# craftsangjae/instance-segmentation-road-project

Measured on AMD Instinct MI355X. Metric: images/sec at 1024x1024 (MaskLab inference hot path, full forward), higher is better.
Workload: dtype f32

## Files before the change

### include/masklab_hip.h

```cpp
#ifndef MASKLAB_HIP_H
#define MASKLAB_HIP_H

#include <stdint.h>

#ifdef __cplusplus
extern "C" {
#endif

#define ML_OK 0
#define ML_E_BADARG (-1)
#define ML_E_LAUNCH (-2)
#define ML_E_NOGPU  (-3)

enum { ML_ACT_NONE = 0, ML_ACT_RELU = 1, ML_ACT_RELU6 = 2, ML_ACT_SIGMOID = 3 };
enum { ML_MATH_F32 = 0, ML_MATH_F16 = 1, ML_MATH_F16S = 2, ML_MATH_F32X3 = 3 };

#define ML_ABI_VERSION 7
int ml_version(void);
const char *ml_last_error(void);
int ml_device_check(void);

typedef struct ml_conv2d_desc {
    const float *in;
    const float *wgt;
    const float *bias;
    const float *residual;
    float *out;
    int32_t B, H, W;
    int32_t in_cstride, in_coff;
    int32_t span;
    int32_t span_pad;
    int32_t cpp_shift;
    int32_t Ho, Wo;
    int32_t KH, KW, stride, dil, pad_t, pad_l;
    int32_t cout;
    int32_t n_pad;
    int32_t out_cstride, out_coff;
    int32_t res_cstride, res_coff;
    int32_t act;
    int32_t group_cin_step;
    int32_t shuffle2x2;
    int32_t tile;
    int32_t math;
    int32_t out_f16;
    int64_t out_bstride;
    const int32_t *live;
    int32_t live_period;
    int32_t reserved1;
    double *gn_partials;
} ml_conv2d_desc;

int ml_conv2d_f32(const ml_conv2d_desc *d, void *stream);

#define ML_CONV_MAX_PROBLEMS 12
int64_t ml_conv2d_workspace_bytes(void);
int ml_conv2d_multi_f32(const ml_conv2d_desc *descs, int32_t n, void *workspace, int64_t workspace_bytes,
                        void *stream);
int ml_conv2d_ntile(int32_t cout, int32_t tile);
int ml_conv2d_launch_ntile(const ml_conv2d_desc *descs, int32_t n, int32_t has_workspace);
int ml_conv2d_launch_mtile(const ml_conv2d_desc *descs, int32_t n, int32_t has_workspace);
int ml_conv2d_uses_pipe(const ml_conv2d_desc *d);
int ml_conv2d_launch_splits(const ml_conv2d_desc *descs, int32_t n, int64_t workspace_bytes, int32_t *splits);
int ml_conv2d_wino_eligible(const ml_conv2d_desc *d);
int ml_conv2d_wino_narrow(const ml_conv2d_desc *d);
int64_t ml_conv2d_gn_min_launch_tiles(void);

#define ML_CONV_WGRAD_MAX_PROBLEMS 8
typedef struct ml_conv2d_wgrad_desc {
    ml_conv2d_desc conv;
    float *dkernel;
    float *dbias;
    const float *add_kernel;
    const float *add_bias;
} ml_conv2d_wgrad_desc;
int ml_conv2d_wgrad_multi_f32(const ml_conv2d_wgrad_desc *descs, int32_t n, void *workspace, int64_t workspace_bytes,
                              void *stream);
int ml_conv2d_wgrad_plan(const ml_conv2d_wgrad_desc *desc, int32_t *slices, int32_t *slice_pixels, int64_t *workspace_bytes);
int ml_conv2d_grad_gather_dy_f32(const float *dy, float *out, int32_t B, int32_t HW, int32_t cout, int32_t dy_cstride,
                                 int64_t dy_bstride, void *stream);

int ml_gconv3x3_f32(const float *in, const float *wgt, const float *bias, float *out,
                    int32_t B, int32_t H, int32_t W, int32_t C, int32_t c, int32_t Ho, int32_t Wo,
                    int32_t stride, int32_t pad_t, int32_t pad_l, int32_t act, void *stream);

int ml_gconv3x3_f16(const void *in, const float *wgt, const float *bias, void *out,
                    int32_t B, int32_t H, int32_t W, int32_t C, int32_t c, int32_t Ho, int32_t Wo,
                    int32_t stride, int32_t pad_t, int32_t pad_l, int32_t act, void *stream);

int ml_gconv3x3_launch_plan(int32_t B, int32_t H, int32_t W, int32_t C, int32_t c, int32_t stride, int32_t Ho, int32_t Wo,
                            int32_t is_half, int32_t plan[6]);

int ml_maxpool3x3s2_f16(const void *in, void *out, int32_t B, int32_t H, int32_t W, int32_t C,
                        int32_t Ho, int32_t Wo, int32_t pad_t, int32_t pad_l, void *stream);
int ml_subsample2_f16(const void *in, void *out, int32_t B, int32_t H, int32_t W, int32_t C, void *stream);
int ml_cast_f16_to_f32(const void *in, float *out, int64_t n, void *stream);
int ml_cast_f32_to_f16(const float *in, void *out, int64_t n, void *stream);
int ml_resize_bilinear_ac_f16(const void *in, const void *add, void *out,
                              int32_t B, int32_t H, int32_t W, int32_t C, int32_t in_cstride, int32_t in_coff,
                              int32_t Ho, int32_t Wo, int32_t add_cstride, int32_t add_coff,
                              int32_t out_cstride, int32_t out_coff, void *stream);
int ml_dwconv3x3_f16(const void *in, const float *wgt, const float *bias, void *out,
                     int32_t B, int32_t H, int32_t W, int32_t C, int32_t in_cstride, int32_t in_coff,
                     int32_t out_cstride, int32_t out_coff, int32_t Ho, int32_t Wo,
                     int32_t stride, int32_t dil, int32_t pad_t, int32_t pad_l, int32_t act, void *stream);
int ml_global_mean_f16(const void *in, void *out, int32_t B, int32_t HW, int32_t C, void *stream);

int ml_stem7x7s2_pool_f16(const float *image, const void *wgt_h, const float *bias, void *out, int32_t B, int32_t H,
                          int32_t W, int32_t Hp, int32_t Wp, void *stream);
int ml_stem7x7s2_pool_f32(const float *image, const float *wgt, const float *bias, float *out, int32_t B, int32_t H,
                          int32_t W, int32_t Hp, int32_t Wp, void *stream);
int ml_stem7x7s2_pool_x3(const float *image, const void *wgt_x3, const float *bias, float *out, int32_t B, int32_t H,
                         int32_t W, int32_t Hp, int32_t Wp, void *stream);

typedef struct ml_deconv_out_problem {
    const float *x, *wd, *bd, *wo_table, *bo;
    float *out;
    int64_t M;
// ... 373 lines not shown
```

### instance-segmentation-road-project_amd/csrc/conv_wino.hip

```cpp
#include "gfx_mem.h"

namespace {

constexpr int WMAXP = ML_CONV_MAX_PROBLEMS;
constexpr int WT = 64;
constexpr int WN = 64;
constexpr int WK = 8;
constexpr int WCHUNK = WK * 32 * 16;
constexpr int WSTEP = 4 * 32 * 16;
constexpr int NSLOT_P = 3;
constexpr int SLOT_P = WT * 16 * 8;
constexpr int NSLOT_W = 4;
constexpr int SLOT_W = 2 * WSTEP;
constexpr int RING_W = NSLOT_P * SLOT_P;
constexpr int LDS_BYTES = (RING_W + NSLOT_W * SLOT_W) * 4;
static_assert(LDS_BYTES == 160 * 1024, "the two rings fill the CU's LDS");
#ifndef WINO_EXP
#define WINO_EXP 0
#endif
constexpr unsigned OOB = 0x80000000u;
constexpr long long SPAN_MAX = 0x7fffff00ll;

struct WProblem {
    ml_conv2d_desc d;
    int TH, TW, T;
    int MB, NB, nchunks;
};

struct WArgs {
    int n;
    int start[WMAXP + 1];
    WProblem p[WMAXP];
};

typedef f32x4 f32x4d __attribute__((aligned(4)));

__device__ __forceinline__ void out_store(float *base, float *ptr, float val) {
#if (WINO_EXP & 8) && defined(__HIP_DEVICE_COMPILE__)
    const __amdgpu_buffer_rsrc_t none = rsrc_bytes(base, 0);
    __builtin_amdgcn_raw_buffer_store_b32(__builtin_bit_cast(unsigned, val), none, (int)((ptr - base) * 4), 0, 0);
#else
    *ptr = val;
#endif
}
__device__ __forceinline__ void out_store(float *base, float *ptr, f32x4 val) {
#if (WINO_EXP & 8) && defined(__HIP_DEVICE_COMPILE__)
    const __amdgpu_buffer_rsrc_t none = rsrc_bytes(base, 0);
    __builtin_amdgcn_raw_buffer_store_b128(__builtin_bit_cast(u32x4, val), none, (int)((ptr - base) * 4), 0, 0);
#else
    *reinterpret_cast<f32x4d *>(ptr) = val;
#endif
}

__device__ __forceinline__ void bt_d_b_op(int k, const float d[16], float t[16], float v[16]) {
    if (k < 16) {
        const int j = k >> 2;
        switch (k & 3) {
            case 0: t[0 * 4 + j] = d[0 * 4 + j] - d[2 * 4 + j]; break;
            case 1: t[1 * 4 + j] = d[1 * 4 + j] + d[2 * 4 + j]; break;
            case 2: t[2 * 4 + j] = d[2 * 4 + j] - d[1 * 4 + j]; break;
            default: t[3 * 4 + j] = d[1 * 4 + j] - d[3 * 4 + j]; break;
        }
    } else {
        const int i = (k - 16) >> 2;
        switch (k & 3) {
            case 0: v[i * 4 + 0] = t[i * 4 + 0] - t[i * 4 + 2]; break;
            case 1: v[i * 4 + 1] = t[i * 4 + 1] + t[i * 4 + 2]; break;
            case 2: v[i * 4 + 2] = t[i * 4 + 2] - t[i * 4 + 1]; break;
            default: v[i * 4 + 3] = t[i * 4 + 1] - t[i * 4 + 3]; break;
        }
    }
}

__global__ void __launch_bounds__(512, 1) conv_wino_kernel(const WArgs args) {
    extern __shared__ __align__(16) float lds[];

    int pi = 0;
    while (pi + 1 < args.n && (int)blockIdx.x >= args.start[pi + 1]) ++pi;
    const WProblem &P = args.p[pi];
    const ml_conv2d_desc &p = P.d;
    const int b = (int)blockIdx.x - args.start[pi];
    const int g = b / (8 * P.NB), rr = b - g * 8 * P.NB;
    const int nt2 = rr >> 3;
    const int mt = g * 8 + (rr & 7);
    if (mt >= P.MB) return;
    if (p.live) {
        const int lv = max(1, *p.live), tpi0 = P.TH * P.TW;
        const int b0 = mt * WT / tpi0, b1 = min(mt * WT + WT, P.T) - 1;
        bool any = false;
        for (int bi = b0; bi <= b1 / tpi0 && !any; ++bi) any = bi % p.live_period < lv;
        if (!any) return;
    }

    const int tid = threadIdx.x, lane = tid & 63;
    const int wave = __builtin_amdgcn_readfirstlane(tid >> 6);
    const int tg = wave & 3, h = wave >> 2;
    const int r = lane & 15, kq = lane >> 4;
    const int tpi = P.TH * P.TW;

    const int gt0 = mt * WT;
    long long base_pix;
    {
        const int bi = gt0 / tpi, rem = gt0 - bi * tpi, ty = rem / P.TW;
        base_pix = ((long long)bi * p.H + max(2 * ty - 1, 0)) * p.W;
    }
    const size_t cstride = (size_t)p.in_cstride;
    const float *pin = p.in + p.in_coff + (size_t)base_pix * cstride;
    int voff_p[4];
    {
        const int rt = (lane >> 1) & 15;
        const int quad = (lane & 1) ^ ((rt >> 2) & 1);
        const int gt = gt0 + (wave >> 1) * 16 + rt;
        int bi = 0, ty = 0, tx = 0;
        if (gt < P.T) {
            bi = gt / tpi;
            const int rem = gt - bi * tpi;
            ty = rem / P.TW;
            tx = rem - ty * P.TW;
        }
#pragma unroll
        for (int i = 0; i < 4; ++i) {
            const int px = 8 * (wave & 1) + 2 * i + (lane >> 5);
            const int y = 2 * ty - 1 + (px >> 2), x = 2 * tx - 1 + (px & 3);
            voff_p[i] = (int)OOB;
            if (gt < P.T && y >= 0 && y < p.H && x >= 0 && x < p.W)
                voff_p[i] = (int)((((long long)bi * p.H + y) * p.W + x - base_pix) * (long long)cstride * 4) + quad * 16;
        }
    }
    const int voff_w = ((wave & 3) * 512 + r * 16 + kq * 4) * 4;
    const float *wsrc = p.wgt + (size_t)(2 * nt2 + (wave >> 2)) * P.nchunks * WCHUNK;
    float *dst_p = lds + (wave >> 1) * 2048 + (wave & 1) * 1024;
    float *dst_w = lds + RING_W + (wave >> 2) * WSTEP + (wave & 3) * 512;
    const int nch = P.nchunks, nsteps = 2 * P.nchunks;
    const bool dead = (2 * nt2 + h) * 32 >= p.cout;

    auto rsrc_p = [&](int j) __attribute__((always_inline)) {
        const bool real = j < nch && !(WINO_EXP & 1);
        return rsrc_bytes(pin + j * 8, real ? (int)OOB : 0);
    };
    auto rsrc_w = [&](int s) __attribute__((always_inline)) {
        const bool real = s < nsteps && !dead && !(WINO_EXP & 2);
        return rsrc_bytes(wsrc + (size_t)s * WSTEP, real ? WSTEP * 4 : 0);
    };

    f32x4 acc[2][16];
#pragma unroll
    for (int t = 0; t < 2; ++t)
#pragma unroll
        for (int q = 0; q < 16; ++q) acc[t][q] = f32x4{0.f, 0.f, 0.f, 0.f};

    const float *pa_lane0 = lds + tg * 2048 + r * 8 + 4 * ((r >> 2) & 1) + kq;
    const float *pa_lane1 = lds + tg * 2048 + r * 8 + 4 * (((r >> 2) & 1) ^ 1) + kq;
    const float *pb_lane = lds + RING_W + h * WSTEP + kq * 512 + r * 4;
    struct Ops {
        float d[16], t[16], v[16];
        f32x4 b[2][4];
    };
    auto read_ops = [&](const float *pa, const float *pb, Ops &o) __attribute__((always_inline)) {
#pragma unroll
        for (int t = 0; t < 2; ++t)
#pragma unroll
            for (int pq = 0; pq < 4; ++pq) o.b[t][pq] = *reinterpret_cast<const f32x4 *>(pb + t * 256 + pq * 64);
#pragma unroll
        for (int px = 0; px < 16; ++px) o.d[px] = pa[px * 128];
    };

    auto step = [&](const Ops &cur, Ops &nxt, const float *pa, const float *pb, const int ndma, auto dma) __attribute__((always_inline)) {
#if WINO_EXP == 4
#pragma unroll
        for (int q = 0; q < ndma; ++q) dma(q);
        __builtin_amdgcn_sched_barrier(0);
#endif
#pragma unroll
        for (int m = 0; m < 32; ++m) {
            const int t = m >> 4, pq = (m >> 2) & 3, e = m & 3;
            acc[t][4 * pq + e] =
                __builtin_amdgcn_mfma_f32_16x16x4f32(cur.b[t][pq][e], cur.v[4 * pq + e], acc[t][4 * pq + e], 0, 0, 0);
            if (m == 3) {
                __builtin_amdgcn_sched_barrier(0);
                read_ops(pa, pb, nxt);
                __builtin_amdgcn_sched_barrier(0);
            }
#if WINO_EXP != 4
            if (m % 6 == 5 && m / 6 < ndma) {
                __builtin_amdgcn_sched_barrier(0);
                dma(m / 6);
                __builtin_amdgcn_sched_barrier(0);
            }
#endif
            if (m >= 16) {
                bt_d_b_op(2 * (m - 16), nxt.d, nxt.t, nxt.v);
                bt_d_b_op(2 * (m - 16) + 1, nxt.d, nxt.t, nxt.v);
                __builtin_amdgcn_sched_barrier(0);
            }
        }
    };

    {
        const __amdgpu_buffer_rsrc_t rp0 = rsrc_p(0), rp1 = rsrc_p(1), rw0 = rsrc_w(0), rw1 = rsrc_w(1), rw2 = rsrc_w(2);
#pragma unroll
        for (int i = 0; i < 4; ++i) lds_dma16(rp0, (char *)(dst_p + i * 256), voff_p[i], 0);
        lds_dma16(rw0, (char *)dst_w, voff_w, 0);
        lds_dma16(rw0, (char *)(dst_w + 256), voff_w + 1024, 0);
#pragma unroll
        for (int i = 0; i < 4; ++i) lds_dma16(rp1, (char *)(dst_p + SLOT_P + i * 256), voff_p[i], 0);
        lds_dma16(rw1, (char *)(dst_w + SLOT_W), voff_w, 0);
        lds_dma16(rw1, (char *)(dst_w + SLOT_W + 256), voff_w + 1024, 0);
        lds_dma16(rw2, (char *)(dst_w + 2 * SLOT_W), voff_w, 0);
        lds_dma16(rw2, (char *)(dst_w + 2 * SLOT_W + 256), voff_w + 1024, 0);
    }
    wait_vmcnt<8>();
    __builtin_amdgcn_s_barrier();

    if (dead) {
        int ps2 = 2 * SLOT_P;
        for (int j = 0; j < nch; ++j) {
            const int w0 = (2 * j) & 3;
            const int wa = ((w0 ^ 2) + 1) * SLOT_W, wb = w0 * SLOT_W;
            asm volatile("s_waitcnt vmcnt(0) lgkmcnt(0)" ::: "memory");
            __builtin_amdgcn_s_barrier();
            const __amdgpu_buffer_rsrc_t rp = rsrc_p(j + 2), rwa = rsrc_w(2 * j + 3), rwb = rsrc_w(2 * j + 4);
#pragma unroll
            for (int q = 0; q < 8; ++q) {
                if (q < 4) lds_dma16(rp, (char *)(dst_p + ps2 + q * 256), voff_p[q], 0);
                else if (q < 6) lds_dma16(rwa, (char *)(dst_w + wa + (q - 4) * 256), voff_w + (q - 4) * 1024, 0);
                else lds_dma16(rwb, (char *)(dst_w + wb + (q - 6) * 256), voff_w + (q - 6) * 1024, 0);
                __builtin_amdgcn_s_sleep(3);
            }
            ps2 = ps2 == 2 * SLOT_P ? 0 : ps2 + SLOT_P;
        }
        wait_vmcnt<0>();
        return;
    }

    Ops oa, ob;
    read_ops(pa_lane0, pb_lane, oa);
#pragma unroll
    for (int k = 0; k < 32; ++k) bt_d_b_op(k, oa.d, oa.t, oa.v);

    int ps0 = 0, ps1 = SLOT_P, ps2 = 2 * SLOT_P;
    for (int j = 0; j < nch; ++j) {
        const int w0 = (2 * j) & 3;
        const int wa = ((w0 ^ 2) + 1) * SLOT_W, wb = w0 * SLOT_W;
        asm volatile("s_waitcnt vmcnt(0) lgkmcnt(0)" ::: "memory");
        __builtin_amdgcn_s_barrier();
        const __amdgpu_buffer_rsrc_t rp = rsrc_p(j + 2), rwa = rsrc_w(2 * j + 3), rwb = rsrc_w(2 * j + 4);
        auto dma = [&](int q) __attribute__((always_inline)) {
            if (q < 4) lds_dma16(rp, (char *)(dst_p + ps2 + q * 256), voff_p[q], 0);
            else if (q < 6) lds_dma16(rwa, (char *)(dst_w + wa + (q - 4) * 256), voff_w + (q - 4) * 1024, 0);
            else lds_dma16(rwb, (char *)(dst_w + wb + (q - 6) * 256), voff_w + (q - 6) * 1024, 0);
        };
        step(oa, ob, pa_lane1 + ps0, pb_lane + (w0 + 1) * SLOT_W, 5, dma);
        step(ob, oa, pa_lane0 + ps1, pb_lane + (w0 ^ 2) * SLOT_W, 3, [&](int q) __attribute__((always_inline)) { dma(q + 5); });
        const int ps = ps0;
        ps0 = ps1;
        ps1 = ps2;
        ps2 = ps;
    }
    wait_vmcnt<0>();

    const int nt = 2 * nt2 + h;
    const bool gn = p.gn_partials != nullptr && !(WINO_EXP & 16);
    double gs[2] = {0.0, 0.0}, gq[2] = {0.0, 0.0};
    long long f0 = 0;
    if (gn) {
        const int bi = gt0 / tpi, rem = gt0 - bi * tpi, ty = rem / P.TW, tx = rem - ty * P.TW;
        f0 = ((long long)(bi * p.Ho + 2 * ty) * p.Wo + 2 * tx) >> 7;
    }
    const float lo = 0.f, hi = (p.act == ML_ACT_RELU6) ? 6.f : 3.402823466e38f;
    const bool clampv = p.act == ML_ACT_RELU || p.act == ML_ACT_RELU6;
    const int gt = gt0 + tg * 16 + r;
    if (gt < P.T) {
        const int bi = gt / tpi, rem = gt - bi * tpi;
        const int ty = rem / P.TW, tx = rem - ty * P.TW;
        const int oy = 2 * ty, ox = 2 * tx;
        const bool y1 = oy + 1 < p.Ho, x1 = ox + 1 < p.Wo;
        const size_t img = p.out_bstride ? (size_t)bi * (size_t)p.out_bstride : (size_t)bi * p.Ho * p.Wo * p.out_cstride;
        const size_t pix0 = (size_t)oy * p.Wo + ox;
        const long long m_flat0 = (long long)(bi * p.Ho + oy) * p.Wo + ox;
#pragma unroll
        for (int t = 0; t < 2; ++t) {
            const int n = nt * 32 + 16 * t + 4 * kq;
            if (n >= p.cout) continue;
            const bool quad = n + 4 <= p.cout;
            f32x4 u[8];
#pragma unroll
            for (int j = 0; j < 4; ++j) {
                u[j] = acc[t][0 * 4 + j] + acc[t][1 * 4 + j] + acc[t][2 * 4 + j];
                u[4 + j] = acc[t][1 * 4 + j] - acc[t][2 * 4 + j] - acc[t][3 * 4 + j];
            }
            f32x4 bv = {0.f, 0.f, 0.f, 0.f};
            if (p.bias) {
                if (quad) bv = *reinterpret_cast<const f32x4d *>(p.bias + n);
                else
#pragma unroll
                    for (int c = 0; c < 3; ++c)
                        if (n + c < p.cout) bv[c] = p.bias[n + c];
            }
            float *o = p.out + img + p.out_coff + n;
#pragma unroll
            for (int a = 0; a < 2; ++a)
#pragma unroll
                for (int c2 = 0; c2 < 2; ++c2) {
                    if ((a && !y1) || (c2 && !x1)) continue;
                    f32x4 val = (c2 ? u[4 * a + 1] - u[4 * a + 2] - u[4 * a + 3] : u[4 * a + 0] + u[4 * a + 1] + u[4 * a + 2]) + bv;
#pragma unroll
                    for (int c = 0; c < 4; ++c) {
                        if (clampv) val[c] = __builtin_amdgcn_fmed3f(val[c], lo, hi);
                        else if (p.act != ML_ACT_NONE) val[c] = ml_apply_act(val[c], p.act);
                    }
                    float *op = o + (pix0 + (size_t)a * p.Wo + c2) * p.out_cstride;
                    if (quad) out_store(p.out, op, val);
// ... 16 lines not shown
        double *lds_gn = reinterpret_cast<double *>(lds);
        __syncthreads();
#pragma unroll
        for (int o = 32; o > 0; o >>= 1) {
#pragma unroll
            for (int f = 0; f < 2; ++f) {
                gs[f] += __shfl_down(gs[f], o, 64);
                gq[f] += __shfl_down(gq[f], o, 64);
            }
        }
        if (lane == 0) {
            lds_gn[wave * 4 + 0] = gs[0]; lds_gn[wave * 4 + 1] = gq[0];
            lds_gn[wave * 4 + 2] = gs[1]; lds_gn[wave * 4 + 3] = gq[1];
        }
        __syncthreads();
        if (tid < 4) {
            const int hh = tid >> 1, ff = tid & 1;
            const int gt1 = gt0 + WT - 1;
            const int bi = gt1 / tpi, rem = gt1 - bi * tpi, ty = rem / P.TW, tx = rem - ty * P.TW;
            const long long f1 = ((long long)(bi * p.Ho + 2 * ty + 1) * p.Wo + 2 * tx + 1) >> 7;
            const long long ft = ff ? f1 : f0;
            const int slot = 2 * nt2 + hh;
            double s = 0.0, q = 0.0;
            for (int w = 0; w < 4; ++w) { s += lds_gn[(hh * 4 + w) * 4 + 2 * ff]; q += lds_gn[(hh * 4 + w) * 4 + 2 * ff + 1]; }
            p.gn_partials[2 * (ft * 4 + slot)] = s;
            p.gn_partials[2 * (ft * 4 + slot) + 1] = q;
        }
    }
}

}

extern "C" int ml_conv2d_wino_eligible(const ml_conv2d_desc *d) {
    if (!d) return 0;
    return d->math == ML_MATH_F32 && d->KH == 3 && d->KW == 3 && d->stride == 1 && d->dil == 1 && d->pad_t == 1 &&
           d->pad_l == 1 && d->Ho == d->H && d->Wo == d->W && d->cpp_shift == 30 && d->group_cin_step == 0 &&
           !d->shuffle2x2 && !d->residual && !d->out_f16 && d->span % 32 == 0 && d->span_pad == d->span &&
           d->cout <= 128 && d->n_pad == 128;
}

extern "C" int ml_conv2d_wino_narrow(const ml_conv2d_desc *d) {
    if (!d || d->live || d->gn_partials) return 0;
    if (d->n_pad != 32 && d->n_pad != 64 && d->n_pad != 96) return 0;
    if (d->cout < 1 || d->cout > d->n_pad || d->cout == 32 || d->cout == 64) return 0;
    ml_conv2d_desc w = *d;
    w.n_pad = 128;
    return ml_conv2d_wino_eligible(&w);
}

int ml_conv2d_wino_gn_ok(const ml_conv2d_desc &d) {
    if (d.Ho % 2 || d.Wo % 2 || d.cout != 128 || d.out_bstride || d.act == ML_ACT_SIGMOID) return 0;
    const long long TH = d.Ho / 2, TW = d.Wo / 2;
    return (64 % TW == 0 || TW % 64 == 0) && (TH * TW) % 64 == 0;
}

int ml_conv2d_wino_launch(const ml_conv2d_desc *descs, int n, hipStream_t s) {
    ML_REQUIRE(n >= 1 && n <= WMAXP, "conv2d (winograd): need 1..%d problems", WMAXP);
    WArgs args;
    args.n = n;
    long long start = 0;
    for (int i = 0; i < n; ++i) {
        const ml_conv2d_desc &d = descs[i];
        ML_REQUIRE(ml_conv2d_wino_eligible(&d),
                   "conv2d: tile = 6 (Winograd F(2x2,3x3)) needs ML_MATH_F32, a 3x3 stride-1 undilated 'same' conv, no "
                   "groups / shuffle / residual / half output, span %% 32 == 0 and n_pad == 128");
        ML_REQUIRE(((d.in_cstride | d.in_coff) & 3) == 0 && ml_aligned16(d.in) && ml_aligned16(d.wgt),
                   "conv2d (winograd): 16-byte aligned input channels and weights");
        if (d.gn_partials)
            ML_REQUIRE(ml_conv2d_wino_gn_ok(d) && !d.live, "conv2d (winograd): gn_partials needs even Ho / Wo, Wo / 2 dividing or a "
                                                "multiple of 64, (Ho / 2) (Wo / 2) %% 64 == 0, cout = 128, dense output");
        WProblem &P = args.p[i];
        P.d = d;
        P.TH = (d.Ho + 1) / 2;
        P.TW = (d.Wo + 1) / 2;
        const long long T = (long long)d.B * P.TH * P.TW;
        ML_REQUIRE(T < (1ll << 30), "conv2d (winograd): too many tiles");
        P.T = (int)T;
        P.MB = (int)((T + WT - 1) / WT);
        P.NB = (d.cout + WN - 1) / WN;
        P.nchunks = d.span_pad / WK;
        const long long span = (2ll * (WT / P.TW + 2) + 2) * d.W * d.in_cstride * 4;
        ML_REQUIRE(span <= SPAN_MAX, "conv2d (winograd): a block's input rows exceed 2 GiB (W x in_cstride too large)");
        args.start[i] = (int)start;
        start += (long long)(P.MB + 7) / 8 * 8 * P.NB;
        ML_REQUIRE(start < (1ll << 31), "conv2d (winograd): grid too large");
    }
    args.start[n] = (int)start;
    long long tiles128 = 0;
    bool any_gn = false;
    for (int i = 0; i < n; ++i) {
        tiles128 += ((long long)descs[i].B * descs[i].Ho * descs[i].Wo + 127) / 128 * (descs[i].n_pad / 128);
        any_gn = any_gn || descs[i].gn_partials != nullptr;
    }
    ML_REQUIRE(!any_gn || tiles128 >= ml_conv2d_gn_min_launch_tiles(),
               "conv2d (winograd): gn_partials needs a launch of ml_conv2d_gn_min_launch_tiles() tiles of 128 x 128");
    static std::atomic<unsigned long long> lds_ok{0};
    if (int rc = ml_ensure_dynamic_lds(reinterpret_cast<const void *>(conv_wino_kernel), LDS_BYTES, lds_ok, "conv2d (winograd)"))
        return rc;
    hipLaunchKernelGGL(conv_wino_kernel, dim3((unsigned)start), dim3(512), LDS_BYTES, s, args);
    ML_CHECK_LAUNCH("conv2d (winograd)");
    return ML_OK;
}
```

### instance-segmentation-road-project_amd/masklab_hip/_lib.py

```python
import ctypes as C
import os

_HERE = os.path.dirname(os.path.abspath(__file__))
LIB_PATH = os.path.join(_HERE, "libmasklab_hip.so")

ABI_VERSION = 7
ACT_NONE, ACT_RELU, ACT_RELU6, ACT_SIGMOID = 0, 1, 2, 3
ACT_BY_NAME = {None: ACT_NONE, "linear": ACT_NONE, "relu": ACT_RELU, "relu6": ACT_RELU6,
               "sigmoid": ACT_SIGMOID}


class ConvDesc(C.Structure):
    _fields_ = [
        ("in_", C.c_void_p), ("wgt", C.c_void_p), ("bias", C.c_void_p),
        ("residual", C.c_void_p), ("out", C.c_void_p),
        ("B", C.c_int32), ("H", C.c_int32), ("W", C.c_int32),
        ("in_cstride", C.c_int32), ("in_coff", C.c_int32),
        ("span", C.c_int32), ("span_pad", C.c_int32), ("cpp_shift", C.c_int32),
        ("Ho", C.c_int32), ("Wo", C.c_int32),
        ("KH", C.c_int32), ("KW", C.c_int32), ("stride", C.c_int32), ("dil", C.c_int32),
        ("pad_t", C.c_int32), ("pad_l", C.c_int32),
        ("cout", C.c_int32), ("n_pad", C.c_int32),
        ("out_cstride", C.c_int32), ("out_coff", C.c_int32),
        ("res_cstride", C.c_int32), ("res_coff", C.c_int32),
# ... 28 lines not shown
class RoiGradLevel(C.Structure):
    _fields_ = [("dy", C.c_void_p), ("add", C.c_void_p), ("dx", C.c_void_p), ("Hf", C.c_int32), ("Wf", C.c_int32),
                ("n_l", C.c_int32), ("reserved", C.c_int32)]


class DeconvOutProblem(C.Structure):
    _fields_ = [("x", C.c_void_p), ("wd", C.c_void_p), ("bd", C.c_void_p), ("wo_table", C.c_void_p),
                ("bo", C.c_void_p), ("out", C.c_void_p), ("M", C.c_int64), ("hw", C.c_int32), ("w", C.c_int32),
                ("rois_per_image", C.c_int32), ("reserved0", C.c_int32), ("out_image_stride", C.c_int64),
                ("out_base", C.c_int64), ("live", C.c_void_p)]


class SeDesc(C.Structure):
    _fields_ = [("x", C.c_void_p), ("out", C.c_void_p), ("w1", C.c_void_p), ("w2", C.c_void_p),
                ("B", C.c_int32), ("HW", C.c_int32), ("C", C.c_int32), ("Hd", C.c_int32),
                ("live", C.c_void_p), ("live_period", C.c_int32), ("reserved", C.c_int32), ("ws_offset", C.c_int64)]


class SeResidualDesc(C.Structure):
    _fields_ = [("x", C.c_void_p), ("shortcut", C.c_void_p), ("w1", C.c_void_p), ("b1", C.c_void_p),
                ("w2", C.c_void_p), ("b2", C.c_void_p), ("scale", C.c_void_p), ("shift", C.c_void_p),
                ("out_act", C.c_void_p), ("out_y", C.c_void_p),
                ("B", C.c_int32), ("HW", C.c_int32), ("C", C.c_int32), ("Hd", C.c_int32),
                ("mode", C.c_int32), ("reserved", C.c_int32)]


class SeBottleneckDesc(C.Structure):
    _fields_ = [("c3", C.c_void_p), ("residual", C.c_void_p), ("w1", C.c_void_p), ("b1", C.c_void_p),
                ("w2", C.c_void_p), ("b2", C.c_void_p), ("out", C.c_void_p),
                ("B", C.c_int32), ("HW", C.c_int32), ("C", C.c_int32), ("Hd", C.c_int32)]


class OptTensor(C.Structure):
    _fields_ = [("p", C.c_void_p), ("g", C.c_void_p), ("m", C.c_void_p), ("v", C.c_void_p), ("n", C.c_int64),
                ("first_chunk", C.c_int64)]


class OptState(C.Structure):
    _fields_ = [("iterations", C.c_int64), ("lr", C.c_float), ("reserved", C.c_int32)]


class OptScalars(C.Structure):
    _fields_ = [("beta_1", C.c_float), ("one_minus_beta_1", C.c_float), ("beta_2", C.c_float), ("one_minus_beta_2", C.c_float),
                ("epsilon", C.c_float), ("lr", C.c_float), ("step", C.c_float), ("wd_lr", C.c_float), ("lr_t", C.c_float),
                ("eta_wd", C.c_float), ("rectified", C.c_int32), ("decays", C.c_int32)]


SE_RES_GATE, SE_RES_BN_RELU = 0, 1
GN_MAX_PROBLEMS = 8
CONV_WGRAD_MAX_PROBLEMS = 8
SE_MAX_PROBLEMS = 8
RESAMPLE_MAX_LEVELS = 8
DECONV_OUT_MAX_PROBLEMS = 4
_i32, _i64, _f32, _f64, _vp = C.c_int32, C.c_int64, C.c_float, C.c_double, C.c_void_p

SIGNATURES = {
    "ml_version": (C.c_int, []),
    "ml_last_error": (C.c_char_p, []),
    "ml_device_check": (C.c_int, []),
    "ml_conv2d_f32": (C.c_int, [C.POINTER(ConvDesc), _vp]),
    "ml_conv2d_ntile": (C.c_int, [_i32, _i32]),
    "ml_conv2d_uses_pipe": (C.c_int, [C.POINTER(ConvDesc)]),
    "ml_conv2d_launch_ntile": (C.c_int, [C.POINTER(ConvDesc), _i32, _i32]),
    "ml_conv2d_launch_mtile": (C.c_int, [C.POINTER(ConvDesc), _i32, _i32]),
    "ml_conv2d_launch_splits": (C.c_int, [C.POINTER(ConvDesc), _i32, _i64, C.POINTER(C.c_int32)]),
    "ml_conv2d_wino_eligible": (C.c_int, [C.POINTER(ConvDesc)]),
    "ml_conv2d_wino_narrow": (C.c_int, [C.POINTER(ConvDesc)]),
    "ml_conv2d_gn_min_launch_tiles": (_i64, []),
    "ml_conv2d_workspace_bytes": (_i64, []),
    "ml_conv2d_multi_f32": (C.c_int, [C.POINTER(ConvDesc), _i32, _vp, _i64, _vp]),
    "ml_conv2d_wgrad_multi_f32": (C.c_int, [C.POINTER(ConvWgradDesc), _i32, _vp, _i64, _vp]),
    "ml_conv2d_wgrad_plan": (C.c_int, [C.POINTER(ConvWgradDesc), C.POINTER(C.c_int32), C.POINTER(C.c_int32), C.POINTER(C.c_int64)]),
    "ml_conv2d_grad_gather_dy_f32": (C.c_int, [_vp, _vp, _i32, _i32, _i32, _i32, _i64, _vp]),
    "ml_deconv2x2_out1x1_f32": (C.c_int, [C.POINTER(DeconvOutProblem), _i32, _i32, _i32, _i32, _i32, _i32, _i32, _vp]),
    "ml_gconv3x3_f32": (C.c_int, [_vp, _vp, _vp, _vp] + [_i32] * 11 + [_vp]),
    "ml_gconv3x3_f16": (C.c_int, [_vp, _vp, _vp, _vp] + [_i32] * 11 + [_vp]),
    "ml_gconv3x3_launch_plan": (C.c_int, [_i32] * 9 + [C.POINTER(C.c_int32)]),
    "ml_maxpool3x3s2_f16": (C.c_int, [_vp, _vp] + [_i32] * 8 + [_vp]),
    "ml_stem7x7s2_pool_f16": (C.c_int, [_vp, _vp, _vp, _vp] + [_i32] * 5 + [_vp]),
    "ml_stem7x7s2_pool_f32": (C.c_int, [_vp, _vp, _vp, _vp] + [_i32] * 5 + [_vp]),
    "ml_stem7x7s2_pool_x3": (C.c_int, [_vp, _vp, _vp, _vp] + [_i32] * 5 + [_vp]),
    "ml_subsample2_f16": (C.c_int, [_vp, _vp] + [_i32] * 4 + [_vp]),
    "ml_cast_f16_to_f32": (C.c_int, [_vp, _vp, _i64, _vp]),
    "ml_cast_f32_to_f16": (C.c_int, [_vp, _vp, _i64, _vp]),
    "ml_resize_bilinear_ac_f16": (C.c_int, [_vp, _vp, _vp] + [_i32] * 12 + [_vp]),
    "ml_dwconv3x3_f16": (C.c_int, [_vp, _vp, _vp, _vp] + [_i32] * 15 + [_vp]),
    "ml_global_mean_f16": (C.c_int, [_vp, _vp, _i32, _i32, _i32, _vp]),
    "ml_groupnorm_chunk_f16": (C.c_int, [_vp, _vp, _vp, _vp, _i32, _i64, _i32, _i32, _f32, _i32, _i32, _i32, _vp, _vp]),
    "ml_roi_crop_resize_f16": (C.c_int, [_vp, _vp, _i32, _i32, _vp, _vp, _vp, _vp] + [_i32] * 10 + [_f32, _f32, _i32, _i32, _vp, _vp]),
    "ml_deconv2x2_out1x1_f16": (C.c_int, [C.POINTER(DeconvOutProblem), _i32, _i32, _i32, _i32, _i32, _i32, _i32, _vp]),
    "ml_dwconv3x3_f32": (C.c_int, [_vp, _vp, _vp, _vp] + [_i32] * 15 + [_vp]),
    "ml_maxpool3x3s2_f32": (C.c_int, [_vp, _vp] + [_i32] * 8 + [_vp]),
    "ml_preprocess_f32": (C.c_int, [_vp, _i32, _vp, _i64, _i32, _i32, C.POINTER(C.c_float), C.POINTER(C.c_float),
                                    C.POINTER(C.c_float), _vp]),
    "ml_groupnorm_workspace_bytes": (_i64, [_i32, _i32]),
    "ml_groupnorm_multi_f32": (C.c_int, [C.POINTER(GnDesc), _i32, _vp, _i64, _vp]),
    "ml_groupnorm_chunk_f32": (C.c_int, [_vp, _vp, _vp, _vp, _i32, _i64, _i32, _i32, _f32, _i32, _i32, _i32, _vp, _vp]),
    "ml_groupnorm_grad_workspace_bytes": (_i64, [_i32, _i32, _i32]),
    "ml_groupnorm_chunk_grad_f32": (C.c_int, [_vp] * 8 + [_i32, _i64, _i32, _i32, _f32, _i32, _i32, _vp, _vp]),
    "ml_groupnorm_chunk_stats_f32": (C.c_int, [_vp, _vp, _i32, _i64, _i32, _i32, _vp, _vp]),
    "ml_groupnorm_grad_multi_f32": (C.c_int, [C.POINTER(GnGradDesc), _i32, _vp, _i64, _vp]),
    "ml_resize_bilinear_ac_f32": (C.c_int, [_vp, _vp, _vp] + [_i32] * 12 + [_vp]),
    "ml_resize_bilinear_ac_grad_workspace_bytes": (_i64, [_i32] * 6),
    "ml_resize_bilinear_ac_grad_f32": (C.c_int, [_vp, _vp, _vp] + [_i32] * 8 + [_vp, _i64, _vp]),
    "ml_global_mean_grad_f32": (C.c_int, [_vp, _vp, _vp, _i32, _i32, _i32, _vp]),
    "ml_global_mean_f32": (C.c_int, [_vp, _vp, _i32, _i32, _i32, _vp]),
    "ml_scale_channels_f32": (C.c_int, [_vp, _vp, _i32, _i32, _i32, _vp]),
    "ml_squeeze_excite_workspace_bytes": (_i64, [_i32, _i32, _i32]),
    "ml_squeeze_excite_f32": (C.c_int, [C.POINTER(SeDesc), _i32, _vp, _i64, _vp]),
    "ml_squeeze_excite_f16": (C.c_int, [C.POINTER(SeDesc), _i32, _vp, _i64, _vp]),
    "ml_se_residual_workspace_bytes": (_i64, [_i32, _i32, _i32]),
    "ml_se_residual_f32": (C.c_int, [C.POINTER(SeResidualDesc), _vp, _i64, _vp]),
    "ml_se_bottleneck_workspace_bytes": (_i64, [_i32, _i32, _i32]),
    "ml_se_bottleneck_f32": (C.c_int, [C.POINTER(SeBottleneckDesc), _vp, _i64, _vp]),
    "ml_se_bottleneck_f16": (C.c_int, [C.POINTER(SeBottleneckDesc), _vp, _i64, _vp]),
    "ml_conv1x1_dual_f32": (C.c_int, [_vp] * 5 + [_i32] * 7 + [_vp]),
    "ml_conv1x1_dual_f16": (C.c_int, [_vp] * 5 + [_i32] * 7 + [_vp]),
    "ml_restore_boxes_f32": (C.c_int, [_vp, _vp, _vp, _i32, _i32, _vp]),
    "ml_detection_workspace_bytes": (_i64, [_i32, _i32, _i32, _i32]),
    "ml_detection_proposal_f32": (C.c_int, [_vp, _vp, _vp, _vp, _vp, _vp, _i32, _i32, _i32, _f32, _f32, _f32, _i32, _vp, _vp]),
# ... 112 lines not shown
```

Measured before the change: 435.2.

## Stage Winograd input patches with shared overlap pixels to cut DMA pieces

Reworks how the Winograd F(2x2,3x3) kernel stages input patches into LDS. Adjacent tiles in a row share their overlapping columns, so each tile stores only its own low half, and the high half is read from the next tile or from a small run-tail area. This can reduce per-chunk patch DMA from four pieces to three when rows are long enough, with the piece count chosen per block at runtime via a templated k-loop. Weight prefetch DMAs are also issued before the patch geometry is computed. The cost is more complex index math (float-reciprocal divisions), two code paths, and a new host-side debug map function for validating the layout.

```diff
diff --git a/include/masklab_hip.h b/include/masklab_hip.h
--- a/include/masklab_hip.h
+++ b/include/masklab_hip.h
@@ -63,6 +63,8 @@
 int ml_conv2d_launch_splits(const ml_conv2d_desc *descs, int32_t n, int64_t workspace_bytes, int32_t *splits);
 int ml_conv2d_wino_eligible(const ml_conv2d_desc *d);
 int ml_conv2d_wino_narrow(const ml_conv2d_desc *d);
+#define ML_WINO_STAGE_MAP_LEN (8 + 2048 + 4 * 64)
+int ml_wino_stage_map(const ml_conv2d_desc *d, int32_t block, int64_t *out);
 int64_t ml_conv2d_gn_min_launch_tiles(void);
 
 #define ML_CONV_WGRAD_MAX_PROBLEMS 8
diff --git a/instance-segmentation-road-project_amd/csrc/conv_wino.hip b/instance-segmentation-road-project_amd/csrc/conv_wino.hip
--- a/instance-segmentation-road-project_amd/csrc/conv_wino.hip
+++ b/instance-segmentation-road-project_amd/csrc/conv_wino.hip
@@ -1,4 +1,5 @@
 #include "gfx_mem.h"
+#include "wino_stage.h"
 
 namespace {
 
@@ -98,50 +99,45 @@
     const int r = lane & 15, kq = lane >> 4;
     const int tpi = P.TH * P.TW;
 
-    const int gt0 = mt * WT;
-    long long base_pix;
-    {
-        const int bi = gt0 / tpi, rem = gt0 - bi * tpi, ty = rem / P.TW;
-        base_pix = ((long long)bi * p.H + max(2 * ty - 1, 0)) * p.W;
-    }
-    const size_t cstride = (size_t)p.in_cstride;
-    const float *pin = p.in + p.in_coff + (size_t)base_pix * cstride;
-    int voff_p[4];
-    {
-        const int rt = (lane >> 1) & 15;
-        const int quad = (lane & 1) ^ ((rt >> 2) & 1);
-        const int gt = gt0 + (wave >> 1) * 16 + rt;
-        int bi = 0, ty = 0, tx = 0;
-        if (gt < P.T) {
-            bi = gt / tpi;
-            const int rem = gt - bi * tpi;
-            ty = rem / P.TW;
-            tx = rem - ty * P.TW;
-        }
-#pragma unroll
-        for (int i = 0; i < 4; ++i) {
-            const int px = 8 * (wave & 1) + 2 * i + (lane >> 5);
-            const int y = 2 * ty - 1 + (px >> 2), x = 2 * tx - 1 + (px & 3);
-            voff_p[i] = (int)OOB;
-            if (gt < P.T && y >= 0 && y < p.H && x >= 0 && x < p.W)
-                voff_p[i] = (int)((((long long)bi * p.H + y) * p.W + x - base_pix) * (long long)cstride * 4) + quad * 16;
-        }
-    }
     const int voff_w = ((wave & 3) * 512 + r * 16 + kq * 4) * 4;
     const float *wsrc = p.wgt + (size_t)(2 * nt2 + (wave >> 2)) * P.nchunks * WCHUNK;
-    float *dst_p = lds + (wave >> 1) * 2048 + (wave & 1) * 1024;
     float *dst_w = lds + RING_W + (wave >> 2) * WSTEP + (wave & 3) * 512;
     const int nch = P.nchunks, nsteps = 2 * P.nchunks;
     const bool dead = (2 * nt2 + h) * 32 >= p.cout;
 
+    auto rsrc_w = [&](int s) __attribute__((always_inline)) {
+        const bool real = s < nsteps && !dead && !(WINO_EXP & 2);
+        return rsrc_bytes(wsrc + (size_t)s * WSTEP, real ? WSTEP * 4 : 0);
+    };
+    {
+        const __amdgpu_buffer_rsrc_t rw0 = rsrc_w(0), rw1 = rsrc_w(1), rw2 = rsrc_w(2);
+        lds_dma16(rw0, (char *)dst_w, voff_w, 0);
+        lds_dma16(rw0, (char *)(dst_w + 256), voff_w + 1024, 0);
+        lds_dma16(rw1, (char *)(dst_w + SLOT_W), voff_w, 0);
+        lds_dma16(rw1, (char *)(dst_w + SLOT_W + 256), voff_w + 1024, 0);
+        lds_dma16(rw2, (char *)(dst_w + 2 * SLOT_W), voff_w, 0);
+        lds_dma16(rw2, (char *)(dst_w + 2 * SLOT_W + 256), voff_w + 1024, 0);
+        __builtin_amdgcn_sched_barrier(0);
+    }
+
+    const WinoStageGeom G = wino_stage_geom(p.H, p.W, P.TH, P.TW, P.T);
+    const WinoStageBlock BG = wino_stage_block(G, mt);
+    const int gt0 = BG.gt0;
+    const int y0 = max(2 * BG.ty0 - 1, 0);
+    const size_t cstride = (size_t)p.in_cstride;
+    const float *pin = p.in + p.in_coff + (size_t)(((long long)BG.bi0 * p.H + y0) * p.W) * cstride;
+    float *dst_p = lds + (wave >> 1) * (WS_ROW_UNITS * 4) + (wave & 1) * 256;
+    auto patch_voff = [&](int i) __attribute__((always_inline)) {
+        const int e = wino_stage_lane_entry(wino_stage_piece_block(wave, i), lane);
+        const WinoStageEntry en = wino_stage_entry(G, BG, e);
+        int bi, y, x;
+        if (!wino_stage_pixel(G, BG, en, wave >> 1, wino_stage_lane_parity(lane), bi, y, x)) return (int)OOB;
+        return (((bi - BG.bi0) * p.H + y - y0) * p.W + x) * (p.in_cstride * 4) + ((lane & 1) ^ en.swz) * 16;
+    };
     auto rsrc_p = [&](int j) __attribute__((always_inline)) {
         const bool real = j < nch && !(WINO_EXP & 1);
         return rsrc_bytes(pin + j * 8, real ? (int)OOB : 0);
     };
-    auto rsrc_w = [&](int s) __attribute__((always_inline)) {
-        const bool real = s < nsteps && !dead && !(WINO_EXP & 2);
-        return rsrc_bytes(wsrc + (size_t)s * WSTEP, real ? WSTEP * 4 : 0);
-    };
 
     f32x4 acc[2][16];
 #pragma unroll
@@ -149,23 +145,28 @@
 #pragma unroll
         for (int q = 0; q < 16; ++q) acc[t][q] = f32x4{0.f, 0.f, 0.f, 0.f};
 
-    const float *pa_lane0 = lds + tg * 2048 + r * 8 + 4 * ((r >> 2) & 1) + kq;
-    const float *pa_lane1 = lds + tg * 2048 + r * 8 + 4 * (((r >> 2) & 1) ^ 1) + kq;
+    const int e_lo = tg * 16 + r;
+    const WinoStageTile tl = wino_stage_tile(G, BG, e_lo);
+    const float *pa_lo0 = lds + wino_stage_unit(e_lo, 0, tl.swz_lo) * 4 + kq;
+    const float *pa_lo1 = lds + wino_stage_unit(e_lo, 1, tl.swz_lo) * 4 + kq;
+    const float *pa_hi0 = lds + wino_stage_unit(tl.hi, 0, tl.swz_hi) * 4 + kq;
+    const float *pa_hi1 = lds + wino_stage_unit(tl.hi, 1, tl.swz_hi) * 4 + kq;
     const float *pb_lane = lds + RING_W + h * WSTEP + kq * 512 + r * 4;
     struct Ops {
         float d[16], t[16], v[16];
         f32x4 b[2][4];
     };
-    auto read_ops = [&](const float *pa, const float *pb, Ops &o) __attribute__((always_inline)) {
+    auto read_ops = [&](const float *pa, const float *pah, const float *pb, Ops &o) __attribute__((always_inline)) {
 #pragma unroll
         for (int t = 0; t < 2; ++t)
 #pragma unroll
             for (int pq = 0; pq < 4; ++pq) o.b[t][pq] = *reinterpret_cast<const f32x4 *>(pb + t * 256 + pq * 64);
 #pragma unroll
-        for (int px = 0; px < 16; ++px) o.d[px] = pa[px * 128];
-    };
-
-    auto step = [&](const Ops &cur, Ops &nxt, const float *pa, const float *pb, const int ndma, auto dma) __attribute__((always_inline)) {
+        for (int px = 0; px < 16; ++px)
+            o.d[px] = (px & 2 ? pah : pa)[(px >> 2) * (WS_ROW_UNITS * 4) + (px & 1) * (WS_PAR_UNITS * 4)];
+    };
+
+    auto step = [&](const Ops &cur, Ops &nxt, const float *pa, const float *pah, const float *pb, const int ndma, auto dma) __attribute__((always_inline)) {
 #if WINO_EXP == 4
 #pragma unroll
         for (int q = 0; q < ndma; ++q) dma(q);
@@ -178,7 +179,7 @@
                 __builtin_amdgcn_mfma_f32_16x16x4f32(cur.b[t][pq][e], cur.v[4 * pq + e], acc[t][4 * pq + e], 0, 0, 0);
             if (m == 3) {
                 __builtin_amdgcn_sched_barrier(0);
-                read_ops(pa, pb, nxt);
+                read_ops(pa, pah, pb, nxt);
                 __builtin_amdgcn_sched_barrier(0);
             }
 #if WINO_EXP != 4
@@ -196,21 +197,27 @@
         }
     };
 
+    auto kloop = [&](auto np_c) __attribute__((always_inline)) {
+    constexpr int NP = decltype(np_c)::value;
+    int voff_p[NP];
+#pragma unroll
+    for (int i = 0; i < NP; ++i) voff_p[i] = patch_voff(i);
     {
-        const __amdgpu_buffer_rsrc_t rp0 = rsrc_p(0), rp1 = rsrc_p(1), rw0 = rsrc_w(0), rw1 = rsrc_w(1), rw2 = rsrc_w(2);
-#pragma unroll
-        for (int i = 0; i < 4; ++i) lds_dma16(rp0, (char *)(dst_p + i * 256), voff_p[i], 0);
-        lds_dma16(rw0, (char *)dst_w, voff_w, 0);
-        lds_dma16(rw0, (char *)(dst_w + 256), voff_w + 1024, 0);
-#pragma unroll
-        for (int i = 0; i < 4; ++i) lds_dma16(rp1, (char *)(dst_p + SLOT_P + i * 256), voff_p[i], 0);
-        lds_dma16(rw1, (char *)(dst_w + SLOT_W), voff_w, 0);
-        lds_dma16(rw1, (char *)(dst_w + SLOT_W + 256), voff_w + 1024, 0);
-        lds_dma16(rw2, (char *)(dst_w + 2 * SLOT_W), voff_w, 0);
-        lds_dma16(rw2, (char *)(dst_w + 2 * SLOT_W + 256), voff_w + 1024, 0);
-    }
-    wait_vmcnt<8>();
+        const __amdgpu_buffer_rsrc_t rp0 = rsrc_p(0), rp1 = rsrc_p(1);
+#pragma unroll
+        for (int i = 0; i < NP; ++i) lds_dma16(rp0, (char *)(dst_p + i * 512), voff_p[i], 0);
+#pragma unroll
+        for (int i = 0; i < NP; ++i) lds_dma16(rp1, (char *)(dst_p + SLOT_P + i * 512), voff_p[i], 0);
+    }
+    wait_vmcnt<NP>();
     __builtin_amdgcn_s_barrier();
+    auto dma_q = [&](int q, int ps2, int wa, int wb, __amdgpu_buffer_rsrc_t rp, __amdgpu_buffer_rsrc_t rwa,
+                     __amdgpu_buffer_rsrc_t rwb) __attribute__((always_inline)) {
+        if (q < NP) {
+            if (!(WINO_EXP & 32) || q < 2) lds_dma16(rp, (char *)(dst_p + ps2 + q * 512), voff_p[q], 0);
+        } else if (q < NP + 2) lds_dma16(rwa, (char *)(dst_w + wa + (q - NP) * 256), voff_w + (q - NP) * 1024, 0);
+        else lds_dma16(rwb, (char *)(dst_w + wb + (q - NP - 2) * 256), voff_w + (q - NP - 2) * 1024, 0);
+    };
 
     if (dead) {
         int ps2 = 2 * SLOT_P;
@@ -221,20 +228,18 @@
             __builtin_amdgcn_s_barrier();
             const __amdgpu_buffer_rsrc_t rp = rsrc_p(j + 2), rwa = rsrc_w(2 * j + 3), rwb = rsrc_w(2 * j + 4);
 #pragma unroll
-            for (int q = 0; q < 8; ++q) {
-                if (q < 4) lds_dma16(rp, (char *)(dst_p + ps2 + q * 256), voff_p[q], 0);
-                else if (q < 6) lds_dma16(rwa, (char *)(dst_w + wa + (q - 4) * 256), voff_w + (q - 4) * 1024, 0);
-                else lds_dma16(rwb, (char *)(dst_w + wb + (q - 6) * 256), voff_w + (q - 6) * 1024, 0);
+            for (int q = 0; q < NP + 4; ++q) {
+                dma_q(q, ps2, wa, wb, rp, rwa, rwb);
                 __builtin_amdgcn_s_sleep(3);
             }
             ps2 = ps2 == 2 * SLOT_P ? 0 : ps2 + SLOT_P;
         }
         wait_vmcnt<0>();
-        return;
+        return false;
     }
 
     Ops oa, ob;
-    read_ops(pa_lane0, pb_lane, oa);
+    read_ops(pa_lo0, pa_hi0, pb_lane, oa);
 #pragma unroll
     for (int k = 0; k < 32; ++k) bt_d_b_op(k, oa.d, oa.t, oa.v);
 
@@ -245,19 +250,18 @@
         asm volatile("s_waitcnt vmcnt(0) lgkmcnt(0)" ::: "memory");
         __builtin_amdgcn_s_barrier();
         const __amdgpu_buffer_rsrc_t rp = rsrc_p(j + 2), rwa = rsrc_w(2 * j + 3), rwb = rsrc_w(2 * j + 4);
-        auto dma = [&](int q) __attribute__((always_inline)) {
-            if (q < 4) lds_dma16(rp, (char *)(dst_p + ps2 + q * 256), voff_p[q], 0);
-            else if (q < 6) lds_dma16(rwa, (char *)(dst_w + wa + (q - 4) * 256), voff_w + (q - 4) * 1024, 0);
-            else lds_dma16(rwb, (char *)(dst_w + wb + (q - 6) * 256), voff_w + (q - 6) * 1024, 0);
-        };
-        step(oa, ob, pa_lane1 + ps0, pb_lane + (w0 + 1) * SLOT_W, 5, dma);
-        step(ob, oa, pa_lane0 + ps1, pb_lane + (w0 ^ 2) * SLOT_W, 3, [&](int q) __attribute__((always_inline)) { dma(q + 5); });
+        auto dma = [&](int q) __attribute__((always_inline)) { dma_q(q, ps2, wa, wb, rp, rwa, rwb); };
+        step(oa, ob, pa_lo1 + ps0, pa_hi1 + ps0, pb_lane + (w0 + 1) * SLOT_W, NP + 1, dma);
+        step(ob, oa, pa_lo0 + ps1, pa_hi0 + ps1, pb_lane + (w0 ^ 2) * SLOT_W, 3, [&](int q) __attribute__((always_inline)) { dma(q + NP + 1); });
         const int ps = ps0;
         ps0 = ps1;
         ps1 = ps2;
         ps2 = ps;
     }
     wait_vmcnt<0>();
+    return true;
+    };
+    if (!(BG.npieces > 3 ? kloop(std::integral_constant<int, 4>{}) : kloop(std::integral_constant<int, 3>{}))) return;
 
     const int nt = 2 * nt2 + h;
     const bool gn = p.gn_partials != nullptr && !(WINO_EXP & 16);
@@ -380,6 +384,42 @@
     if (d.Ho % 2 || d.Wo % 2 || d.cout != 128 || d.out_bstride || d.act == ML_ACT_SIGMOID) return 0;
     const long long TH = d.Ho / 2, TW = d.Wo / 2;
     return (64 % TW == 0 || TW % 64 == 0) && (TH * TW) % 64 == 0;
+}
+
+extern "C" int ml_wino_stage_map(const ml_conv2d_desc *d, int block, int64_t *out) {
+    ML_REQUIRE(d && out, "ml_wino_stage_map: null argument");
+    ml_conv2d_desc w = *d;
+    if (ml_conv2d_wino_narrow(&w)) w.n_pad = 128;
+    ML_REQUIRE(ml_conv2d_wino_eligible(&w), "ml_wino_stage_map: not a problem of the Winograd kernel");
+    const long long T = (long long)d->B * ((d->Ho + 1) / 2) * ((d->Wo + 1) / 2);
+    ML_REQUIRE(T >= 1 && T < (1ll << 30), "ml_wino_stage_map: too many tiles");
+    const WinoStageGeom G = wino_stage_geom(d->H, d->W, (d->Ho + 1) / 2, (d->Wo + 1) / 2, (int)T);
+    const int MB = (G.T + WT - 1) / WT;
+    ML_REQUIRE(block >= 0 && block < MB, "ml_wino_stage_map: block %d of %d", block, MB);
+    const WinoStageBlock BG = wino_stage_block(G, block);
+    out[0] = BG.npieces, out[1] = BG.nruns, out[2] = BG.nentries, out[3] = WS_ROW_UNITS, out[4] = WS_PAR_UNITS;
+    out[5] = WS_SLOT_UNITS, out[6] = std::min(WT, G.T - BG.gt0), out[7] = 0;
+    int64_t *units = out + 8, *tiles = out + 8 + WS_SLOT_UNITS;
+    for (int u = 0; u < WS_SLOT_UNITS; ++u) units[u] = -2;
+    for (int wave = 0; wave < 8; ++wave)
+        for (int i = 0; i < BG.npieces; ++i)
+            for (int lane = 0; lane < 64; ++lane) {
+                const int kb = wino_stage_piece_block(wave, i), e = wino_stage_lane_entry(kb, lane);
+                const WinoStageEntry en = wino_stage_entry(G, BG, e);
+                int bi, y, x;
+                int64_t v = -1;
+                if (wino_stage_pixel(G, BG, en, wave >> 1, wino_stage_lane_parity(lane), bi, y, x))
+                    v = (((int64_t)bi * d->H + y) * d->W + x) * d->in_cstride + d->in_coff + 4 * ((lane & 1) ^ en.swz);
+                units[(wave >> 1) * WS_ROW_UNITS + kb * 64 + lane] = v;
+            }
+    for (int lt = 0; lt < WT; ++lt) {
+        const WinoStageTile tl = wino_stage_tile(G, BG, lt);
+        for (int q = 0; q < 2; ++q) {
+            tiles[4 * lt + q] = wino_stage_unit(lt, q, tl.swz_lo);
+            tiles[4 * lt + 2 + q] = wino_stage_unit(tl.hi, q, tl.swz_hi);
+        }
+    }
+    return ML_OK;
 }
 
 int ml_conv2d_wino_launch(const ml_conv2d_desc *descs, int n, hipStream_t s) {
diff --git a/instance-segmentation-road-project_amd/csrc/wino_stage.h b/instance-segmentation-road-project_amd/csrc/wino_stage.h
--- /dev/null
+++ b/instance-segmentation-road-project_amd/csrc/wino_stage.h
@@ -0,0 +1,117 @@
+#pragma once
+
+constexpr int WS_TILES = 64;
+constexpr int WS_ROW_UNITS = 512;
+constexpr int WS_PAR_UNITS = 32;
+constexpr int WS_SLOT_UNITS = 2048;
+constexpr int WS_BLOCK_ENTRIES = 16;
+constexpr int WS_PIECE_ENTRIES = 32;
+
+struct WinoStageGeom {
+    int H, W, TH, TW, T;
+    float rcp_tw, rcp_th;
+};
+
+struct WinoStageBlock {
+    int gt0;
+    int row0, off;
+    int bi0, ty0;
+    int nruns;
+    int ms, spread, klast;
+    int nentries, npieces;
+};
+
+__host__ __device__ inline int ws_div(int n, int d, float rcp_d) {
+    return d >= 256 ? (n >= d ? 1 : 0) : (int)(((float)n + 0.5f) * rcp_d);
+}
+__host__ __device__ inline float ws_rcp(int d) {
+#if defined(__HIP_DEVICE_COMPILE__)
+    return __builtin_amdgcn_rcpf((float)d);
+#else
+    return 1.0f / (float)d;
+#endif
+}
+__host__ __device__ inline WinoStageGeom wino_stage_geom(int H, int W, int TH, int TW, int T) {
+    return WinoStageGeom{H, W, TH, TW, T, ws_rcp(TW), ws_rcp(TH)};
+}
+
+__host__ __device__ inline WinoStageBlock wino_stage_block(const WinoStageGeom &g, int mt) {
+    WinoStageBlock b;
+    b.gt0 = mt * WS_TILES;
+    b.row0 = b.gt0 / g.TW;
+    b.off = b.gt0 - b.row0 * g.TW;
+    b.bi0 = b.row0 / g.TH;
+    b.ty0 = b.row0 - b.bi0 * g.TH;
+    b.nruns = ws_div(b.off + WS_TILES - 1, g.TW, g.rcp_tw) + 1;
+    b.ms = (g.TW & 1) ? 2 : (g.TW & 2) ? 1 : 0;
+    b.klast = (b.nruns - 1 + (1 << b.ms) - 1) >> b.ms;
+    b.spread = 4 * b.klast + 1 <= WS_PIECE_ENTRIES;
+    b.nentries = WS_TILES + (b.spread ? 4 * b.klast + 1 : b.nruns);
+    b.npieces = (b.nentries + WS_PIECE_ENTRIES - 1) / WS_PIECE_ENTRIES;
+    return b;
+}
+
+__host__ __device__ inline int wino_stage_run_end(const WinoStageGeom &g, const WinoStageBlock &b, int rho) {
+    const int end = (rho + 1) * g.TW - b.off;
+    return end < WS_TILES ? end : WS_TILES;
+}
+__host__ __device__ inline int wino_stage_tail(const WinoStageGeom &g, const WinoStageBlock &b, int rho) {
+    if (!b.spread) return rho;
+    return rho == b.nruns - 1 ? 4 * b.klast : 4 * (rho >> b.ms) + (wino_stage_run_end(g, b, rho) & 3);
+}
+
+struct WinoStageEntry {
+    int rho, c, swz;
+    bool used;
+};
+__host__ __device__ inline WinoStageEntry wino_stage_entry(const WinoStageGeom &g, const WinoStageBlock &b, int e) {
+    WinoStageEntry en;
+    if (e < WS_TILES) {
+        en.rho = ws_div(e + b.off, g.TW, g.rcp_tw);
+        en.c = e + b.off - en.rho * g.TW;
+        en.swz = (e >> 2) & 1;
+        en.used = true;
+        return en;
+    }
+    const int t = e - WS_TILES;
+    int rho = -1;
+    if (!b.spread) rho = t < b.nruns ? t : -1;
+    else if ((t >> 2) == b.klast) rho = (t & 3) == 0 ? b.nruns - 1 : -1;
+    else
+        for (int j = 0; j < 4; ++j) {
+            const int cand = ((t >> 2) << b.ms) + j;
+            if (j < (1 << b.ms) && cand < b.nruns - 1 && (wino_stage_run_end(g, b, cand) & 3) == (t & 3)) rho = cand;
+        }
+    en.used = rho >= 0;
+    en.rho = en.used ? rho : 0;
+    const int end = wino_stage_run_end(g, b, en.rho);
+    en.c = end + b.off - en.rho * g.TW;
+    en.swz = (end >> 2) & 1;
+    return en;
+}
+
+__host__ __device__ inline bool wino_stage_pixel(const WinoStageGeom &g, const WinoStageBlock &b, const WinoStageEntry &en, int a,
+                                                 int par, int &bi, int &y, int &x) {
+    const int trow = b.ty0 + en.rho, di = ws_div(trow, g.TH, g.rcp_th);
+    bi = b.bi0 + di;
+    y = 2 * (trow - di * g.TH) - 1 + a;
+    x = 2 * en.c - 1 + par;
+    return en.used && ((long long)b.row0 + en.rho) * g.TW < g.T && y >= 0 && y < g.H && x >= 0 && x < g.W;
+}
+
+struct WinoStageTile {
+    int hi, swz_lo, swz_hi;
+};
+__host__ __device__ inline WinoStageTile wino_stage_tile(const WinoStageGeom &g, const WinoStageBlock &b, int lt) {
+    const int rho = ws_div(lt + b.off, g.TW, g.rcp_tw);
+    WinoStageTile t;
+    t.swz_lo = (lt >> 2) & 1;
+    t.swz_hi = ((lt + 1) >> 2) & 1;
+    t.hi = lt + 1 == wino_stage_run_end(g, b, rho) ? WS_TILES + wino_stage_tail(g, b, rho) : lt + 1;
+    return t;
+}
+
+__host__ __device__ inline int wino_stage_unit(int e, int q, int swz) { return (e >> 4) * 64 + (e & 15) * 2 + (q ^ swz); }
+__host__ __device__ inline int wino_stage_piece_block(int wave, int i) { return 2 * i + (wave & 1); }
+__host__ __device__ inline int wino_stage_lane_entry(int block, int lane) { return WS_BLOCK_ENTRIES * block + ((lane >> 1) & 15); }
+__host__ __device__ inline int wino_stage_lane_parity(int lane) { return lane >> 5; }
diff --git a/instance-segmentation-road-project_amd/masklab_hip/_lib.py b/instance-segmentation-road-project_amd/masklab_hip/_lib.py
--- a/instance-segmentation-road-project_amd/masklab_hip/_lib.py
+++ b/instance-segmentation-road-project_amd/masklab_hip/_lib.py
@@ -104,6 +104,7 @@
 SE_MAX_PROBLEMS = 8
 RESAMPLE_MAX_LEVELS = 8
 DECONV_OUT_MAX_PROBLEMS = 4
+WINO_STAGE_MAP_LEN = 8 + 2048 + 4 * 64
 _i32, _i64, _f32, _f64, _vp = C.c_int32, C.c_int64, C.c_float, C.c_double, C.c_void_p
 
 SIGNATURES = {
@@ -118,6 +119,7 @@
     "ml_conv2d_launch_splits": (C.c_int, [C.POINTER(ConvDesc), _i32, _i64, C.POINTER(C.c_int32)]),
     "ml_conv2d_wino_eligible": (C.c_int, [C.POINTER(ConvDesc)]),
     "ml_conv2d_wino_narrow": (C.c_int, [C.POINTER(ConvDesc)]),
+    "ml_wino_stage_map": (C.c_int, [C.POINTER(ConvDesc), _i32, C.POINTER(C.c_int64)]),
     "ml_conv2d_gn_min_launch_tiles": (_i64, []),
     "ml_conv2d_workspace_bytes": (_i64, []),
     "ml_conv2d_multi_f32": (C.c_int, [C.POINTER(ConvDesc), _i32, _vp, _i64, _vp]),
```

Result: no change. 433.5 (-0.4%).
